# faithokamoto/panman

Measured on AMD Instinct MI355X. Metric: Fitch-Sankoff site*node updates/sec (fitch mode), higher is better.
Workload: dtype u32 bit-planes (16-bit one-hot state sets); 1 GPU; N* fitch: 1000000 leaves x 30000 sites random-join tree (one MI355X, north-star size); tree=random-join, leaves=1000000, nodes=1999999, sites=30000, sites_per_gpu=30000, parallelism=column shards x1, one all-gather of per-site score/root, gather=none (1 GPU), mutations_total=125584115, launch=hipGraph replay, per-level kernels

## Files before the change

### include/panman_gpu.h

```cpp
#ifndef PANMAN_GPU_H
#define PANMAN_GPU_H

#include <stdint.h>

#ifdef __cplusplus
extern "C" {
#endif

#define PM_OK 0
#define PM_ERR_ARG (-1)
#define PM_ERR_OOM (-2)
#define PM_ERR_HIP (-3)
#define PM_ERR_UNSUPPORTED (-4)
#define PM_ERR_STATE (-5)

#define PM_MODE_FITCH 0
#define PM_MODE_SANKOFF 1
#define PM_MODE_BLOCK_FITCH 2
#define PM_MODE_BLOCK_SANKOFF 3

#define PM_MUT_NS 0
#define PM_MUT_ND 1
#define PM_MUT_NI 2

typedef struct pm_ctx pm_ctx;

typedef struct pm_tree {
    int32_t num_nodes;
    int32_t root;
    const int32_t* child_offsets;
    const int32_t* child_index;
} pm_tree;

typedef struct pm_mut {
    uint32_t node;
    uint32_t site_info;
} pm_mut;

int pm_create(int device, pm_ctx** out);
void pm_destroy(pm_ctx* ctx);
int pm_warmup(int device);
const char* pm_last_error(const pm_ctx* ctx);
int pm_set_stream(pm_ctx* ctx, void* hip_stream);
#define PM_OPT_VIRTUAL 2
#define PM_OPT_GRAPH 3
#define PM_OPT_SUBTREE 6
#define PM_OPT_NARROW 7
#define PM_OPT_GROUP_WAVES 8
#define PM_OPT_GROUP_LEVELS 9
#define PM_OPT_UP_GROUP 10
#define PM_OPT_RECORD_CAP 12
#define PM_OPT_SUB_DOWN 13
#define PM_OPT_PLAIN_UP 14
#define PM_OPT_NT_LOADS 16
#define PM_OPT_CLUSTER 17
int pm_set_option(pm_ctx* ctx, int option, int64_t value);
int pm_set_profiling(pm_ctx* ctx, int enable);

int pm_tree_upload(pm_ctx* ctx, const pm_tree* tree);

int pm_leaves_upload(pm_ctx* ctx, int64_t num_sites, const uint8_t* codes4, int64_t row_stride,
                     const int32_t* node_row, const uint8_t* present, int64_t present_stride);

int pm_sites_upload(pm_ctx* ctx, const uint8_t* consensus4, const uint8_t* forced4);

int pm_run(pm_ctx* ctx, int mode);

int pm_mutation_count(pm_ctx* ctx, int64_t* count);
int pm_mutations_fetch(pm_ctx* ctx, pm_mut* out, int64_t cap, int64_t* count);
int pm_site_results(pm_ctx* ctx, int32_t* score, uint8_t* root_code);
int pm_site_results_device(pm_ctx* ctx, void* score_device, void* root_code_device);
int pm_kernel_times(pm_ctx* ctx, double* ms, int64_t* launches, int classes);

#define PM_COMM_ID_BYTES 128
int pm_comm_unique_id(uint8_t* id, int64_t len);
int pm_comm_init_rank(pm_ctx* ctx, const uint8_t* id, int nranks, int rank);
int pm_comm_init_all(pm_ctx* const* ctxs, int n);
int pm_run_gather(pm_ctx* ctx, int mode, int64_t total_sites, int64_t site_begin, void* score_device,
                  void* root_device);
int pm_multi_run(pm_ctx* const* ctxs, int n, int mode, const int64_t* site_begin, int64_t total_sites,
                 int32_t* score, uint8_t* root_code);
int pm_shard_range(int rank, int ranks, int64_t total_sites, int64_t* begin, int64_t* end);
int pm_pack_site_results(pm_ctx* ctx, int64_t site_begin, int64_t per, void* chunk_device);
int pm_unpack_site_results(pm_ctx* ctx, const void* all_device, int64_t per, int ranks, int64_t total_sites,
                           void* score_device, void* root_device);
int pm_chunk_entries(int64_t total_sites, int ranks, int64_t* per);
int pm_chunk_pack(int64_t site_begin, int64_t count, const int32_t* score, const uint8_t* root, int64_t per,
                  uint64_t* chunk);
int pm_chunk_unpack(const uint64_t* all, int64_t per, int ranks, int64_t total_sites, int32_t* score,
                    uint8_t* root);

int pm_design_bytes(pm_ctx* ctx, double* out, int n);
int pm_gather_probe(int device, int64_t lanes, int stride_bytes, int reps, double* ms_per_launch);
int pm_memory_footprint(pm_ctx* ctx, int64_t* out, int n);
const char* pm_build_id(void);
int pm_stream_copy_rate(int device, int64_t bytes, int reps, double* gbs);
int pm_stream_write_rate(int device, int64_t bytes, int reps, double* gbs);

void pm_phase_reset(void);
int64_t pm_phase_report(char* buf, int64_t len);

char* pm_msa_build(const char* newick, const char* msa_text, const char* reference, int mode, int device);
void pm_free(void* p);
int pm_msa_to_panman(const char* newick, const char* msa_text, const char* reference, int mode, int device,
                     const char* out_path, char* err, int64_t err_len);
int pm_msa_to_panman_multi(const char* newick, const char* msa_text, const char* reference, int mode,
                           const int* devices, int num_devices, const char* out_path, char* err, int64_t err_len);

// ... 82 lines not shown
```

### panman_amd/csrc/pm_fitch.hip

```cpp
#include "pm_kernels.h"

#if PM_NT_LOADS
#define launch_fitch launch_fitch_nt
#define warm_fitch warm_fitch_nt
#endif

namespace pm {
namespace {

#ifndef PM_LEAFY_WAVES
#define PM_LEAFY_WAVES 6
#endif
#ifndef PM_SUB_LEAFY_WAVES
#define PM_SUB_LEAFY_WAVES 4
#endif
#ifndef PM_SUB_UP_WAVES
#define PM_SUB_UP_WAVES 4
#endif
#ifndef PM_GROUP_UP_WAVES
#define PM_GROUP_UP_WAVES 4
#endif
template <bool AP, bool LEAFY, bool SUB = false, bool GROUP = false, bool PLAIN = false>
__device__ __forceinline__ void fitch_up_node(const UpArgs& a, const NodeDesc& d, int32_t gi, int tile, int lane) {
    constexpr bool SS = SUB && !PLAIN;
// ... 793 lines not shown
                else if (ap && c->group_waves > 0) hipLaunchKernelGGL((k_down_band<Mode::kFitch, true, false, true>), dim3(tiles), dim3(kBandBlock), 0, c->stream, dn, tab, base, d, d1);
                else if (ap) hipLaunchKernelGGL((k_down_band<Mode::kFitch, true>), dim3(tiles), dim3(kBandBlock), 0, c->stream, dn, tab, base, d, d1);
                else if (c->group_waves > 0) hipLaunchKernelGGL((k_down_band<Mode::kFitch, false, false, true>), dim3(tiles), dim3(kBandBlock), 0, c->stream, dn, tab, base, d, d1);
                else hipLaunchKernelGGL((k_down_band<Mode::kFitch, false>), dim3(tiles), dim3(kBandBlock), 0, c->stream, dn, tab, base, d, d1);
                timer_end(c, 1);
                d = d1 - 1;
                continue;
            }
        }
        dn.desc = down_desc + down_off[d];
        dn.count = down_off[d + 1] - down_off[d];
        if (dn.count == 0) continue;
        const bool dense = sub ? ht.down_dense_k : virt && ht.down_dense_v;
        dn.dense_base = !dense ? -1 : sub ? ht.down_dense_base_k[d] : down_off[d];
        auto narrow_down = [&](int l) { return c->narrow_max > 0 && down_off[l + 1] - down_off[l] <= c->narrow_max; };
        auto band_at = [&](int l) { return narrow_down(l) && l + 1 < D && narrow_down(l + 1); };
        int g = 1;
        int64_t items = dn.count;
        while (!block && c->group_waves > 0 && g < std::min(c->group_levels, kGroupLevels) && d + g < D) {
            const int32_t ng = down_off[d + g + 1] - down_off[d + g];
            if (ng == 0 || (items + ng) * tiles > c->group_waves || band_at(d + g)) break;
            items += ng;
            ++g;
        }
        if (g > 1) {
            for (int k = 0; k < 4; ++k) {
                const int l = std::min(d + k, d + g - 1);
                if (k > 0) dn.split[k - 1] = k < g ? down_off[d + k] - down_off[d] : (int32_t)items;
                dn.dense_g[k] = !dense ? -1 : sub ? ht.down_dense_base_k[l] : down_off[l];
            }
            dn.count = (int32_t)items;
            const dim3 grid = wave_grid(dn.count, tiles);
            timer_begin(c, 1);
            if (sub_down && dense) hipLaunchKernelGGL((k_down<Mode::kFitch, true, true, true, true>), grid, dim3(kBlock), 0, c->stream, dn);
            else if (sub_down) hipLaunchKernelGGL((k_down<Mode::kFitch, true, false, true, true>), grid, dim3(kBlock), 0, c->stream, dn);
            else if (ap && dense) hipLaunchKernelGGL((k_down<Mode::kFitch, true, true, false, true>), grid, dim3(kBlock), 0, c->stream, dn);
            else if (ap) hipLaunchKernelGGL((k_down<Mode::kFitch, true, false, false, true>), grid, dim3(kBlock), 0, c->stream, dn);
            else hipLaunchKernelGGL((k_down<Mode::kFitch, false, false, false, true>), grid, dim3(kBlock), 0, c->stream, dn);
            timer_end(c, 1);
            d += g - 1;
            continue;
        }
        const dim3 grid = wave_grid(dn.count, tiles);
        timer_begin(c, 1);
        if (block && ap) hipLaunchKernelGGL((k_down<Mode::kBlockFitch, true, false>), grid, dim3(kBlock), 0, c->stream, dn);
        else if (block) hipLaunchKernelGGL((k_down<Mode::kBlockFitch, false, false>), grid, dim3(kBlock), 0, c->stream, dn);
        else if (sub_down && dense) hipLaunchKernelGGL((k_down<Mode::kFitch, true, true, true>), grid, dim3(kBlock), 0, c->stream, dn);
        else if (sub_down) hipLaunchKernelGGL((k_down<Mode::kFitch, true, false, true>), grid, dim3(kBlock), 0, c->stream, dn);
        else if (ap && dense) hipLaunchKernelGGL((k_down<Mode::kFitch, true, true>), grid, dim3(kBlock), 0, c->stream, dn);
        else if (ap) hipLaunchKernelGGL((k_down<Mode::kFitch, true, false>), grid, dim3(kBlock), 0, c->stream, dn);
        else hipLaunchKernelGGL((k_down<Mode::kFitch, false, false>), grid, dim3(kBlock), 0, c->stream, dn);
        timer_end(c, 1);
    }
    const int32_t tail_skip = sub_down ? ht.num_tail_s : 0;
    const int32_t tail_total = (sub ? ht.num_tail_k : virt ? ht.num_tail_v : ht.num_tail) - tail_skip;
    if (tail_total > 0) {
        DownArgs t = dn;
        t.tail = (sub ? dt.tail_desc_k : virt ? dt.tail_desc_v : dt.tail_desc) + tail_skip;
        t.count = tail_total;
        t.num_s = sub && !sub_down ? ht.num_tail_s : 0;
        t.sbase = ht.sbase;
        t.sub_planes = c->sub_planes;
        const dim3 grid = wave_grid(t.count, tiles);
        timer_begin(c, 5);
        if (sub) hipLaunchKernelGGL((k_tail<Mode::kFitch, true, true>), grid, dim3(kBlock), 0, c->stream, t);
        else if (block && ap) hipLaunchKernelGGL((k_tail<Mode::kBlockFitch, true>), grid, dim3(kBlock), 0, c->stream, t);
        else if (block) hipLaunchKernelGGL((k_tail<Mode::kBlockFitch, false>), grid, dim3(kBlock), 0, c->stream, t);
        else if (ap) hipLaunchKernelGGL((k_tail<Mode::kFitch, true>), grid, dim3(kBlock), 0, c->stream, t);
        else hipLaunchKernelGGL((k_tail<Mode::kFitch, false>), grid, dim3(kBlock), 0, c->stream, t);
        timer_end(c, 5);
    }
    return hipGetLastError();
}

#if !PM_NT_LOADS
hipError_t launch_score(pm_ctx* c) {
    hipError_t e = hipMemsetAsync(c->score, 0, sizeof(int32_t) * c->num_sites, c->stream);
    if (e != hipSuccess) return e;
    const bool use_lds = c->num_sites * 4 <= 150 * 1024;
    const int spb = kShards >= 1024 ? kShards / 256 : 4;
    const int blocks = (kShards + spb - 1) / spb;
    const size_t lds = use_lds ? (size_t)c->num_sites * 4 : 0;
    timer_begin(c, 2);
    hipLaunchKernelGGL(k_site_score, dim3(blocks), dim3(kScoreBlock), lds, c->stream, c->recs, c->shard_cnt,
                       c->shard_cap, (uint32_t)c->ht.root, c->score, c->num_sites, spb, use_lds);
    timer_end(c, 2);
    return hipGetLastError();
}

#endif

hipError_t warm_fitch() {
    hipFuncAttributes at;
    return hipFuncGetAttributes(&at, reinterpret_cast<const void*>(&k_fitch_up_wide<true>));
}

}
```

### panman_amd/csrc/pm_host.cpp

```cpp
#include <algorithm>
#include <chrono>
#include <cstdio>
#include <cstdlib>
#include <random>
#include <cstring>
#include <numeric>
#include <string>
#include <vector>

#include "pm_internal.h"

namespace pm {

int fail(pm_ctx* c, int code, const std::string& msg) {
    if (c) c->err = msg;
    return code;
}

int hip_fail(pm_ctx* c, hipError_t e, const char* what) {
    return fail(c, PM_ERR_HIP, std::string(what) + ": " + hipGetErrorString(e));
}

namespace {

// ... 152 lines not shown
            if ((e = malloc_or_release(c, reinterpret_cast<void**>(&c->upm), need)) != hipSuccess)
                return fail(c, PM_ERR_OOM, std::string("up slots: ") + hipGetErrorString(e));
            c->upm_bytes = need;
        }
    }
    if (!fitch) {
        const size_t parts = (size_t)std::max(c->ht.part_off.empty() ? 0 : c->ht.part_off.back(),
                                              std::max(c->ht.part_off_v.empty() ? 0 : c->ht.part_off_v.back(),
                                                       std::max(c->ht.part_off_k.empty() ? 0 : c->ht.part_off_k.back(),
                                                                c->ht.part_off_gs.empty() ? 0 : c->ht.part_off_gs.back())));
        const size_t need = parts * kPartPlanes * wpad * sizeof(uint32_t);
        if (need > c->sk_parts_bytes) {
            dev_free(c->sk_parts);
            if ((e = malloc_or_release(c, reinterpret_cast<void**>(&c->sk_parts), need)) != hipSuccess)
                return fail(c, PM_ERR_OOM, std::string("Sankoff part counters: ") + hipGetErrorString(e));
            c->sk_parts_bytes = need;
        }
    }
    if (!c->shard_cnt && (e = dev_alloc(&c->shard_cnt, kShards)) != hipSuccess)
        return fail(c, PM_ERR_OOM, "shard counters");
    if (c->shard_cap == 0) {
        const double nodes = (double)c->dt.num_internal + c->dt.num_leaves;
        const double guess = std::max(65536.0, 0.01 * nodes * (double)c->num_sites);
        const int64_t cap = c->record_cap > 0 ? c->record_cap : (int64_t)(guess * 1.5 / kShards) + 256;
        if ((e = malloc_or_release(c, reinterpret_cast<void**>(&c->recs), sizeof(pm_mut) * (size_t)cap * kShards)) != hipSuccess)
            return fail(c, PM_ERR_OOM, std::string("mutation records: ") + hipGetErrorString(e));
        c->shard_cap = cap;
    }
    return PM_OK;
}

bool nt_policy(const pm_ctx* c) {
    if (c->nt_loads >= 0) return c->nt_loads != 0;
    const std::vector<int32_t>& off = c->ht.down_level_off;
    int64_t widest = 0;
    for (size_t l = 0; l + 1 < off.size(); ++l) widest = std::max<int64_t>(widest, off[l + 1] - off[l]);
    return widest * (wpad_of(c) / kWave) >= 65536;
}

hipError_t launch_all(pm_ctx* c, int mode) {
    const bool sankoff = mode == PM_MODE_SANKOFF || mode == PM_MODE_BLOCK_SANKOFF;
    const bool block = mode == PM_MODE_BLOCK_FITCH || mode == PM_MODE_BLOCK_SANKOFF;
    const bool nt = nt_policy(c);
    phase_add("run.nt_loads", nt ? 1.0 : 0.0);
    hipError_t e = sankoff ? (nt ? launch_sankoff_nt(c, block) : launch_sankoff(c, block))
                           : (nt ? launch_fitch_nt(c, block) : launch_fitch(c, block));
    if (e == hipSuccess) e = launch_score(c);
    return e;
}

uint64_t graph_key_of(const pm_ctx* c, int mode) {
    const uint64_t parts[] = {(uint64_t)mode, (uint64_t)c->virtual_leaf_parents, (uint64_t)c->subtree_form,
                              (uint64_t)c->narrow_max, (uint64_t)c->group_waves, (uint64_t)c->group_levels, (uint64_t)c->up_group,
                              (uint64_t)c->sub_down, (uint64_t)c->plain_up, (uint64_t)c->plain_min_waves, (uint64_t)c->cluster,
                              (uint64_t)(uintptr_t)c->upm,
                              (uint64_t)(uintptr_t)c->sk_parts,
                              (uint64_t)c->leaves_all_present, (uint64_t)c->has_forced, (uint64_t)c->num_sites,
                              (uint64_t)c->shard_cap, (uint64_t)(uintptr_t)c->recs, (uint64_t)(uintptr_t)c->sets,
                              (uint64_t)(uintptr_t)c->cmask, (uint64_t)(uintptr_t)c->root_final,
                              (uint64_t)(uintptr_t)c->leaf_planes, (uint64_t)(uintptr_t)c->leaf_present,
                              (uint64_t)(uintptr_t)c->leaf_flag, (uint64_t)(uintptr_t)c->cons,
                              (uint64_t)(uintptr_t)c->forced, (uint64_t)(uintptr_t)c->score,
                              (uint64_t)(uintptr_t)c->root_code, (uint64_t)(uintptr_t)c->shard_cnt,
                              (uint64_t)(uintptr_t)c->sub_planes, (uint64_t)nt_policy(c),
                              (uint64_t)(uintptr_t)c->dt.child_off, (uint64_t)(uintptr_t)c->stream};
    uint64_t h = 1469598103934665603ull;
    for (uint64_t v : parts) h = (h ^ v) * 1099511628211ull;
    return h | 1;
}

int run_once(pm_ctx* c, int mode) {
    hipError_t e;
    if (!c->use_graph) {
        e = launch_all(c, mode);
        if (e != hipSuccess) return hip_fail(c, e, "parsimony launch");
    } else {
        const uint64_t key = graph_key_of(c, mode);
        if (key != c->graph_key) {
            drop_graph(c);
            const bool prof = c->profiling;
            c->profiling = false;
            hipGraph_t g = nullptr;
            e = hipStreamBeginCapture(c->stream, hipStreamCaptureModeThreadLocal);
            if (e == hipSuccess) {
                const hipError_t le = launch_all(c, mode);
                e = hipStreamEndCapture(c->stream, &g);
                if (e == hipSuccess) e = le;
            }
            c->profiling = prof;
            if (e == hipSuccess) e = hipGraphInstantiate(&c->graph_exec, g, nullptr, nullptr, 0);
            if (g) (void)hipGraphDestroy(g);
            if (e != hipSuccess) {
                drop_graph(c);
                return hip_fail(c, e, "graph capture");
            }
            c->graph_key = key;
        }
        timer_begin(c, 4);
        e = hipGraphLaunch(c->graph_exec, c->stream);
        timer_end(c, 4);
        if (e != hipSuccess) return hip_fail(c, e, "graph launch");
    }
    c->ran = true;
    c->last_mode = mode;
    return PM_OK;
}

// ... 164 lines not shown
    free_columns(c);
    free_tree(c->dt);
    free_replay(c);
    comm_release(c);
    free_hostio(c);
    for (auto& v : c->timers)
        for (auto& t : v) {
            (void)hipEventDestroy(t.a);
            (void)hipEventDestroy(t.b);
        }
    if (c->side) (void)hipStreamSynchronize(c->side);
    if (c->ev_fork) (void)hipEventDestroy(c->ev_fork);
    if (c->ev_join) (void)hipEventDestroy(c->ev_join);
    if (c->side) (void)hipStreamDestroy(c->side);
    if (c->own_stream) (void)hipStreamDestroy(c->own_stream);
    delete c;
}

const char* pm_last_error(const pm_ctx* c) { return c ? c->err.c_str() : "null context"; }

int pm_set_stream(pm_ctx* c, void* s) {
    if (!c) return PM_ERR_ARG;
    c->stream = s ? reinterpret_cast<hipStream_t>(s) : c->own_stream;
    return PM_OK;
}

int pm_set_option(pm_ctx* c, int option, int64_t value) {
    if (!c) return PM_ERR_ARG;
    if (option == PM_OPT_SUBTREE) {
        c->subtree_form = value != 0;
        return PM_OK;
    }
    if (option == PM_OPT_VIRTUAL) {
        c->virtual_leaf_parents = value != 0;
        return PM_OK;
    }
    if (option == PM_OPT_NARROW) {
        if (value < 0 || value > 1024) return fail(c, PM_ERR_ARG, "PM_OPT_NARROW: 0..1024 items per level");
        c->narrow_max = (int32_t)value;
        return PM_OK;
    }
    if (option == PM_OPT_UP_GROUP) {
        c->up_group = value != 0;
        return PM_OK;
    }
    if (option == PM_OPT_PLAIN_UP) {
        if (value < 0) return fail(c, PM_ERR_ARG, "PM_OPT_PLAIN_UP: 0, 1 or a wave threshold >= 2");
        c->plain_up = value != 0;
        c->plain_min_waves = value >= 2 ? value : 0;
        return PM_OK;
    }
    if (option == PM_OPT_SUB_DOWN) {
        c->sub_down = value != 0;
        return PM_OK;
    }
    if (option == PM_OPT_GROUP_WAVES) {
        if (value < 0) return fail(c, PM_ERR_ARG, "PM_OPT_GROUP_WAVES: >= 0 waves");
        c->group_waves = value;
        return PM_OK;
    }
    if (option == PM_OPT_GROUP_LEVELS) {
        if (value < 2 || value > 4) return fail(c, PM_ERR_ARG, "PM_OPT_GROUP_LEVELS: 2 to 4");
        c->group_levels = (int32_t)value;
        return PM_OK;
    }
    if (option == PM_OPT_RECORD_CAP) {
        if (value < 1 || value > ((int64_t)1 << 31)) return fail(c, PM_ERR_ARG, "PM_OPT_RECORD_CAP: 1 .. 2^31 records per shard");
        if (c->stream) (void)hipStreamSynchronize(c->stream);
        drop_graph(c);
        dev_free(c->recs);
        c->shard_cap = 0;
        c->record_cap = value;
        c->ran = false;
        return PM_OK;
    }
    if (option == PM_OPT_NT_LOADS) {
        if (value < -1 || value > 1) return fail(c, PM_ERR_ARG, "PM_OPT_NT_LOADS: -1 (by level size), 0 or 1");
        c->nt_loads = (int32_t)value;
        return PM_OK;
    }
    if (option == PM_OPT_CLUSTER) {
        if (value < 0 || value > ((int64_t)1 << 30)) return fail(c, PM_ERR_ARG, "PM_OPT_CLUSTER: 0, 1 or a level size >= 2");
        c->cluster = value != 0;
        c->cluster_max_level = value == 0 ? 0 : value == 1 ? kClMaxLevel : (int32_t)value;
        c->cluster_chain = value == 1;
        return PM_OK;
    }
    if (option == PM_OPT_GRAPH) {
        c->use_graph = value != 0;
        if (!c->use_graph) drop_graph(c);
        return PM_OK;
    }
    return fail(c, PM_ERR_ARG, "unknown option");
}

int pm_set_profiling(pm_ctx* c, int enable) {
    if (!c) return PM_ERR_ARG;
    c->profiling = enable != 0;
    for (auto& u : c->timers_used) u = 0;
    return PM_OK;
}

int pm_tree_upload(pm_ctx* c, const pm_tree* t) {
    const bool timing = std::getenv("PM_UPLOAD_TIMING") != nullptr;
    auto t_last = std::chrono::steady_clock::now();
    auto upload_phase = [&](const char* what) {
// ... 979 lines not shown
```

### panman_amd/csrc/pm_internal.h

```cpp
#pragma once

#include <hip/hip_runtime.h>

#include <chrono>
#include <cstdint>
#include <functional>
#include <string>
#include <vector>

#include "../../include/panman_gpu.h"

namespace pm {

constexpr int kWave = 64;
constexpr int kWavesPerBlock = 4;
constexpr int kBlock = kWave * kWavesPerBlock;
#ifndef PM_SHARDS
#define PM_SHARDS 1024
#endif
constexpr int kShards = PM_SHARDS;
constexpr int kClasses = 6;
constexpr int kDegreeClasses = 4;
#ifndef PM_CX_COMPACT
#define PM_CX_COMPACT 0
// ... 156 lines not shown
    std::vector<int32_t> up_degree[4];
    std::vector<int32_t> up_level_off_k, up_class_off_k, down_level_off_k, down_dense_base_k;
    std::vector<uint8_t> up_leafy_k;
    std::vector<int32_t> up_level_off_g, up_class_off_g;
    std::vector<uint8_t> up_leafy_g, up_recomp_g;
    std::vector<int32_t> up_plain_g, up_plain_gs;
    std::vector<int32_t> up_level_off_gs, up_class_off_gs;
    std::vector<uint8_t> up_leafy_gs, up_recomp_gs;
    bool down_dense_k = false;
    int32_t up_items_k = 0, up_items_g = 0, up_items_gs = 0;
    int64_t num_sshape = 0;
    std::vector<uint8_t> sshape;
    int32_t num_tail_k = 0;
    int32_t num_tail_s = 0;
    int32_t sbase = -1;
    int64_t lvl_up[5] = {0, 0, 0, 0, 0}, lvl_down[3] = {0, 0, 0}, lvl_base_k = 0;
    ClusterPlan cl;
};

int plan_clusters(const HostTree& ht, const std::vector<int32_t>& up_order_k, const std::vector<int32_t>& child_enc_k,
                  const std::vector<int32_t>& parent_dense, const std::vector<int32_t>& vleaf, int32_t max_level,
                  bool chain_check, ClusterPlan& out);
bool plan_cluster_down(const HostTree& ht, const std::vector<int32_t>& down_order_k, const std::vector<NodeDesc>& down_desc_k,
                       const std::vector<int32_t>& child_enc_k, ClusterPlan& cl);

struct Timer {
    hipEvent_t a = nullptr, b = nullptr;
};

}

namespace pm { struct ReplayState; }

struct pm_ctx {
    int device = 0;
    hipStream_t stream = nullptr;
    hipStream_t own_stream = nullptr;
    hipStream_t side = nullptr;
    hipEvent_t ev_fork = nullptr, ev_join = nullptr;
    std::string err;

    pm::HostTree ht;
    pm::DevTree dt;
    size_t tree_bytes = 0;
    bool has_tree = false;
    int32_t max_degree = 0;
    bool virtual_leaf_parents = true;
    bool subtree_form = true;
    int32_t narrow_max = 16;
    int64_t group_waves = 32768;
    int32_t group_levels = 4;
    bool up_group = true;
    bool sub_down = false;
    bool plain_up = true;
    int64_t plain_min_waves = 0;
    bool cluster = true;
    int32_t cluster_max_level = pm::kClMaxLevel;
    bool cluster_chain = true;

    int64_t num_sites = 0;
    int32_t words = 0;
    uint4* leaf_planes = nullptr;
    uint32_t* leaf_present = nullptr;
    uint8_t* leaf_flag = nullptr;
    uint4* cons = nullptr;
    uint4* forced = nullptr;
    bool has_forced = false;
    bool has_leaves = false;
    bool leaves_all_present = false;
    bool has_sites = false;

    uint32_t* sets = nullptr;
    size_t sets_bytes = 0;
    uint64_t* cmask = nullptr;
    size_t cmask_bytes = 0;
    uint64_t* upm = nullptr;
    size_t upm_bytes = 0;
    uint4* finals = nullptr;
    size_t finals_bytes = 0;
    uint32_t* sk_parts = nullptr;
    size_t sk_parts_bytes = 0;
    uint4* root_final = nullptr;
    pm_mut* recs = nullptr;
    int64_t shard_cap = 0;
    int64_t record_cap = 0;
    uint32_t* shard_cnt = nullptr;
    uint4* sub_planes = nullptr;
    size_t sub_planes_bytes = 0;
    bool sub_planes_ok = false;
    int32_t* score = nullptr;
    uint8_t* root_code = nullptr;
    bool ran = false;
    int last_mode = -1;

    bool profiling = false;
    std::vector<pm::Timer> timers[pm::kClasses];
    size_t timers_used[pm::kClasses] = {0, 0, 0, 0, 0, 0};

    bool use_graph = false;
    int32_t nt_loads = -1;
    hipGraphExec_t graph_exec = nullptr;
    uint64_t graph_key = 0;

    pm::ReplayState* replay = nullptr;

    void* comm = nullptr;
// ... 149 lines not shown
```

### panman_amd/csrc/pm_kernels.h

```cpp
#pragma once

#include "pm_bits.h"
#include "pm_internal.h"

#ifndef PM_NT_LOADS
#define PM_NT_LOADS 0
#endif
#if PM_NT_LOADS
#define PM_KNS kern_nt
#else
#define PM_KNS kern
#endif

namespace pm {
inline namespace PM_KNS {

enum class Mode { kFitch, kSankoff, kBlockFitch };

#ifndef PM_TILE_FAST
#define PM_TILE_FAST 1
#endif
__device__ __forceinline__ void wave_item(int wave, int32_t tiles, int32_t& item, int& tile) {
#if PM_TILE_FAST
    const int32_t g = (int32_t)blockIdx.x * kWavesPerBlock + wave;
// ... 1113 lines not shown
        r.H = r.F;
    } else {
        const uint4 D = k.L3;
        const uint32_t ia = ~code_ne(A, Cc) | ~code_ne(A, D), ib = ~code_ne(B, Cc) | ~code_ne(B, D), nz = ia | ib;
        const uint32_t hit = (nz & ((ePa & ia) | (ePb & ib))) | (~nz & (ePa | ePb | ePc | ~code_ne(P, D)));
        const uint4 mcd = min4(Cc, D);
        r.F = sel4(hit, P, sel4(nz, sel4(ia & ib, mab, sel4(ia, A, B)), min4(mab, mcd)));
        r.H = sel4(~code_ne(r.F, Cc) | ~code_ne(r.F, D), r.F, mcd);
    }
    r.G = sel4(~code_ne(r.F, A) | ~code_ne(r.F, B), r.F, mab);
    return r;
}

__device__ __forceinline__ uint4 cherry_final_sankoff(const uint4& A, const uint4& B, const uint4& F) {
    const uint4 mab = min4(A, B);
    const uint4 open = sel4(~code_ne(F, A) | ~code_ne(F, B), F, min4(mab, F));
    return sel4(~code_ne(A, B), A, open);
}

__device__ __forceinline__ SubFinals subtree_finals_sankoff(const Kid& k, int sh, const uint4& P) {
    const uint4 A = k.L0, B = k.L1, Cc = k.L2;
    const uint4 mab = min4(A, B);
    const uint32_t pX = ~code_ne(P, A) | ~code_ne(P, B);
    SubFinals r;
    if (sh == 1) {
        const uint32_t inx = ~code_ne(Cc, A) | ~code_ne(Cc, B);
        const uint4 f_in = sel4(pX & code_less(&P.x, &Cc.x), P, Cc);
        const uint4 f_out = sel4(pX | ~code_ne(P, Cc), P, min4(min4(mab, Cc), P));
        r.F = sel4(inx, f_in, f_out);
        r.H = r.F;
    } else {
        const uint4 D = k.L3;
        const uint4 mcd = min4(Cc, D);
        const uint32_t ia = ~code_ne(A, Cc) | ~code_ne(A, D), ib = ~code_ne(B, Cc) | ~code_ne(B, D), nz = ia | ib;
        const uint32_t pY = ~code_ne(P, Cc) | ~code_ne(P, D);
        const uint32_t p_z0 = (~code_ne(P, A) & ia) | (~code_ne(P, B) & ib);
        const uint4 low = sel4(ia & ib, mab, sel4(ia, A, B));
        const uint4 f_nz = sel4(p_z0 | ((pX ^ pY) & code_less(&P.x, &low.x)), P, low);
        const uint4 f_z = sel4(pX | pY, P, min4(min4(mab, mcd), P));
        r.F = sel4(nz, f_nz, f_z);
        r.H = cherry_final_sankoff(Cc, D, r.F);
    }
    r.G = cherry_final_sankoff(A, B, r.F);
    return r;
}

template <class Args>
__device__ __forceinline__ void emit_code(const Args& a, Emit& em, int lane, uint32_t node, uint32_t D, uint32_t site0,
                                          const uint4& c, const uint4& pc) {
    const uint32_t p4[4] = {pc.x, pc.y, pc.z, pc.w};
    emit_stream(a, em, lane, node, D, site0, c.x, c.y, c.z, c.w, p4);
}

template <Mode M, class Args>
__device__ __forceinline__ void subtree_emit(const Args& a, Emit& em, int lane, const int32_t* id, int32_t ix, int32_t iy,
                                             const Kid& k, int sh, uint32_t valid, const uint32_t* Fn, uint32_t site0) {
    const uint4 P = make_uint4(Fn[0], Fn[1], Fn[2], Fn[3]);
    const SubFinals f = M == Mode::kSankoff ? subtree_finals_sankoff(k, sh, P) : subtree_finals(k, sh, P);
    const uint32_t msk = valid & k.m0;
    emit_code(a, em, lane, (uint32_t)id[0], msk & code_ne(f.F, P), site0, f.F, P);
    emit_code(a, em, lane, (uint32_t)ix, msk & code_ne(f.G, f.F), site0, f.G, f.F);
    emit_code(a, em, lane, (uint32_t)id[1], msk & code_ne(k.L0, f.G), site0, k.L0, f.G);
    emit_code(a, em, lane, (uint32_t)id[2], msk & code_ne(k.L1, f.G), site0, k.L1, f.G);
    const uint4 pc = sh == 1 ? f.F : f.H;
    emit_code(a, em, lane, (uint32_t)id[3], msk & code_ne(k.L2, pc), site0, k.L2, pc);
    if (sh == 2) {
        emit_code(a, em, lane, (uint32_t)iy, msk & code_ne(f.H, f.F), site0, f.H, f.F);
        emit_code(a, em, lane, (uint32_t)id[4], msk & code_ne(k.L3, f.H), site0, k.L3, f.H);
    }
}

template <Mode M, class Args>
__device__ __forceinline__ void kid_emit(const Args& a, Emit& em, int lane, const Kid& k, uint32_t id0, uint32_t id1,
                                         uint32_t id2, uint32_t valid, const uint32_t* Fn, uint32_t site0) {
    if (k.enc < 0) {
        emit_stream(a, em, lane, id0, valid & k.m0 & diff4(k.L0, Fn), site0, k.L0.x, k.L0.y, k.L0.z, k.L0.w, Fn);
        return;
    }
    if (M == Mode::kBlockFitch || !(k.enc & kVirtualBit)) return;
    uint32_t low[4] = {0, 0, 0, 0}, have = 0, hit = 0;
    virt_fold(k.L0, k.m0, Fn, low, have, hit);
    virt_fold(k.L1, k.m1, Fn, low, have, hit);
    if (M == Mode::kSankoff) {
        const uint32_t z1_has_fn =
            (k.m0 ^ k.m1) |
            (k.m0 & k.m1 & ((k.L0.x ^ k.L1.x) | (k.L0.y ^ k.L1.y) | (k.L0.z ^ k.L1.z) | (k.L0.w ^ k.L1.w)));
        const uint32_t take = z1_has_fn & code_less(Fn, low);
#pragma unroll
        for (int j = 0; j < 4; ++j) low[j] = bsel(take, Fn[j], low[j]);
    }
    uint32_t F[4];
#pragma unroll
    for (int j = 0; j < 4; ++j) F[j] = bsel(hit, Fn[j], low[j]);
    const uint32_t self = have & valid & ((F[0] ^ Fn[0]) | (F[1] ^ Fn[1]) | (F[2] ^ Fn[2]) | (F[3] ^ Fn[3]));
    emit_stream(a, em, lane, id0, self, site0, F[0], F[1], F[2], F[3], Fn);
    emit_stream(a, em, lane, id1, valid & k.m0 & diff4(k.L0, F), site0, k.L0.x, k.L0.y, k.L0.z, k.L0.w, F);
    if (k.vl.y >= 0)
        emit_stream(a, em, lane, id2, valid & k.m1 & diff4(k.L1, F), site0, k.L1.x, k.L1.y, k.L1.z, k.L1.w, F);
}

__device__ __forceinline__ uint32_t final_slot(const RecMask& m) {
    return (uint32_t)__builtin_popcountll(m.s) + lanes_below(m.x);
}

__device__ __forceinline__ uint4 rec_final(const uint4* p, const RecMask& m, int lane, const uint4* cons, int64_t word) {
    const uint4* src = ((m.x >> lane) & 1ull) ? p + final_slot(m)
                                              : ((m.s >> lane) & 1ull) ? p + lanes_below(m.s) : cons + word;
    return *src;
}

template <int REC>
__device__ __forceinline__ uint4 parent_final(const DownArgs& a, int32_t parent, const RecMask& m, int tile, int lane,
                                              int64_t word) {
    if (parent == a.root_dense) return a.root_final[word];
    const RecMask pm{m.px, m.ps, 0, 0, 0};
    return rec_final(a.sets + ((size_t)parent * a.tiles + tile) * REC, pm, lane, a.cons, word);
}

template <int REC>
__device__ __forceinline__ uint4 node_final(const DownArgs& a, int32_t node, int tile, int lane, int64_t word) {
    if (node == a.root_dense) return a.root_final[word];
// ... 151 lines not shown
        kid_emit<M>(a, em, lane, kids[1], kids[1].id0, kids[1].id1, kids[1].id2, valid, F, site0);
    }
    emit_flush<M != Mode::kSankoff>(a, em, lane);
}

template <Mode M, bool AP, bool DENSE, bool SUB = false, bool GROUP = false>
#ifndef PM_SK_GROUP_WAVES
#define PM_SK_GROUP_WAVES 7
#endif
#ifndef PM_DOWN_WAVES
#define PM_DOWN_WAVES 8
#endif
#ifndef PM_SK_DOWN_WAVES
#define PM_SK_DOWN_WAVES 6
#endif
__global__ __launch_bounds__(kBlock, GROUP ? (M == Mode::kSankoff ? PM_SK_GROUP_WAVES : SUB ? PM_SUB_DOWN_WAVES : 8) : SUB ? PM_SUB_DOWN_WAVES : (M == Mode::kFitch && AP) ? PM_DOWN_WAVES : (M == Mode::kSankoff && AP) ? PM_SK_DOWN_WAVES : 1) void k_down(DownArgs a) {
    __shared__ uint4 stage[kWavesPerBlock][kEntryQuads];
    const int wave = __builtin_amdgcn_readfirstlane(threadIdx.x >> 6), lane = threadIdx.x & 63;
    int32_t item;
    int tile;
    wave_item(wave, a.tiles, item, tile);
    if (item >= a.count) return;
    const NodeDesc& d = a.desc[item];
    const int gen = !GROUP ? 0 : (item >= a.split[0]) + (item >= a.split[1]) + (item >= a.split[2]);
    const int32_t first = gen == 0 ? 0 : a.split[gen > 0 ? gen - 1 : 0];
    const int32_t n = !DENSE ? d.node : (GROUP ? a.dense_g[gen] : a.dense_base) + (item - first);
    down_node<M, AP, SUB, GROUP>(a, d, n, (uint32_t)item, tile, lane, stage[wave], gen);
}

template <Mode M, bool AP, bool SUB = false, bool GROUP = false>
__global__ __launch_bounds__(kBandBlock) void k_down_band(DownArgs a, const int32_t* level_off, const int32_t* dense_base,
                                                          int32_t d0, int32_t d1) {
    __shared__ uint4 stage[kBandWaves][kEntryQuads];
    const int wave = __builtin_amdgcn_readfirstlane(threadIdx.x >> 6), lane = threadIdx.x & 63;
    const int tile = blockIdx.x;
    constexpr int G = GROUP ? kGroupLevels : 1;
    for (int32_t l0 = d0; l0 < d1; l0 += G) {
        const int32_t l1 = min(l0 + G, d1);
        for (int32_t i = level_off[l0] + wave; i < level_off[l1]; i += kBandWaves) {
            int32_t l = l0;
            while (l + 1 < l1 && i >= level_off[l + 1]) ++l;
            const NodeDesc& d = a.desc[i];
            const int32_t base = dense_base ? dense_base[l] : -1;
            down_node<M, AP, SUB, GROUP>(a, d, base >= 0 ? base + (i - level_off[l]) : d.node, (uint32_t)i, tile, lane,
                                         stage[wave], l - l0);
        }
        __syncthreads();
    }
}

#ifndef PM_TAIL_WAVES
#define PM_TAIL_WAVES 6
#endif
template <Mode M, bool AP, bool SUB = false>
__global__ __launch_bounds__(kBlock, SUB ? PM_TAIL_WAVES : 1) void k_tail(DownArgs a) {
    __shared__ uint4 stage[kWavesPerBlock][kEntryQuads];
    const int wave = __builtin_amdgcn_readfirstlane(threadIdx.x >> 6), lane = threadIdx.x & 63;
    int32_t item;
    int tile;
    wave_item(wave, a.tiles, item, tile);
    if (item >= a.count) return;
    const TailDesc& t = a.tail[item];
    const int64_t word = (int64_t)tile * kWave + lane;
    const uint32_t valid = valid_mask(a, word);
    constexpr int REC = M == Mode::kSankoff ? kSankoffRec : kFitchRec;
    RecMask pm;
    bool proot;
    if (SUB && item < a.num_s) {
        const uint64_t* q = a.cmask + kMaskWords * ((size_t)(a.sbase + item) * a.tiles + tile);
        pm = RecMask{q[3], q[4], q[5], 0, 0};
        if (pm.d == 0) return;
        proot = t.parent == a.root_dense;
    } else {
        proot = t.parent == a.root_dense;
        pm = rec_mask(a.cmask, (size_t)t.parent * a.tiles + tile);
        if (leaf_rule<M, AP>(t.enc)) pm.d = pm.x;
        if (!proot && pm.d == 0) return;
    }
    const size_t prec = (size_t)t.parent * a.tiles + tile;
    const bool dirty = proot || ((pm.d >> lane) & 1ull);
    Kid k;
    if (SUB && item < a.num_s) {
        k.enc = t.enc;
        k.L0 = k.L1 = k.L2 = k.L3 = make_uint4(0, 0, 0, 0);
        k.m0 = k.m1 = 0;
        const uint4* q = sub_word(a.sub_planes, item, a.wpad, word);
        if (dirty) {
            k.L0 = q[0];
            k.L1 = q[1];
            k.L2 = q[2];
            k.m0 = k.m1 = ~0u;
        }
        if (dirty && kid_shape(t.enc) == 2) k.L3 = q[3];
    } else {
        kid_fetch<M, AP, SUB, false>(a, t.enc, make_int4(t.vl[0], t.vl[1], t.vl[2], t.vl[3]), word, dirty, k);
    }
    const uint4* fsrc = proot ? a.root_final + word
                              : ((pm.x >> lane) & 1ull) ? a.sets + prec * REC + final_slot(pm)
                              : ((pm.s >> lane) & 1ull) ? a.sets + prec * REC + lanes_below(pm.s) : a.cons + word;
    uint4 q = make_uint4(0, 0, 0, 0);
    if (dirty) q = *fsrc;
    const uint32_t F[4] = {q.x, q.y, q.z, q.w};
    Emit em{stage[wave], shard_of((uint32_t)item, tile), 0u, 0u};
    const uint32_t site0 = (uint32_t)(word * 32);
    if (SUB && kid_shape(t.enc)) subtree_emit<M>(a, em, lane, t.id, t.ix, t.iy, k, kid_shape(t.enc), valid, F, site0);
    else kid_emit<M>(a, em, lane, k, (uint32_t)t.id[0], (uint32_t)t.id[1], (uint32_t)t.id[2], valid, F, site0);
    emit_flush<M != Mode::kSankoff>(a, em, lane);
}

struct ClArgs {
    const NodeDesc* items;
    const int32_t* wg_off;
    const int32_t* slot_of;
    const int32_t* pslot;
// ... 241 lines not shown
```

### panman_amd/engine.py

```python
from __future__ import annotations

import ctypes as C

import numpy as np

from ._lib import MODE_BLOCK_FITCH, MODE_BLOCK_SANKOFF, MODE_FITCH, MODE_SANKOFF, Mut, PanmanError, Summary, Tree, load

CLUSTER_DEFAULT = 1

__all__ = ["Engine", "msa_build", "random_join_tree", "pack_codes", "MODE_FITCH", "MODE_SANKOFF"]


def pack_codes(codes: np.ndarray) -> np.ndarray:
    codes = np.ascontiguousarray(codes, dtype=np.uint8)
    if codes.ndim == 1:
        return pack_codes(codes[None, :])[0]
    rows, s = codes.shape
    if s % 2:
        codes = np.concatenate([codes, np.zeros((rows, 1), np.uint8)], axis=1)
    return np.ascontiguousarray(codes[:, 0::2] | (codes[:, 1::2] << 4))


def random_join_tree(leaves: int, seed: int = 1):
    lib = load()
# ... 162 lines not shown
    dv = (C.c_int * len(devices))(*devices)
    n = C.c_int64(0)
    err = C.create_string_buffer(512)
    rc = lib.pm_fasta_multi_fd(C.byref(st), int(aligned), dv, len(devices), int(fd), C.byref(n), err, len(err))
    del keep
    if rc != 0:
        raise PanmanError(f"pm_fasta_multi_fd failed ({rc}): {err.value.decode(errors='replace')}")
    return n.value


class Engine:
    def __init__(self, device: int = 0):
        self.lib = load()
        self.ctx = C.c_void_p()
        rc = self.lib.pm_create(device, C.byref(self.ctx))
        if rc != 0:
            raise PanmanError(f"pm_create({device}) failed ({rc}): no usable HIP device")
        self.num_sites = 0

    def close(self):
        if self.ctx:
            self.lib.pm_destroy(self.ctx)
            self.ctx = C.c_void_p()

    def __del__(self):
        try:
            self.close()
        except Exception:
            pass

    def _check(self, rc: int, what: str):
        if rc != 0:
            msg = self.lib.pm_last_error(self.ctx)
            raise PanmanError(f"{what}: rc={rc}: {msg.decode() if msg else ''}")

    def set_stream(self, stream_handle: int):
        self._check(self.lib.pm_set_stream(self.ctx, C.c_void_p(stream_handle)), "pm_set_stream")

    def set_virtual(self, on: bool):
        self._check(self.lib.pm_set_option(self.ctx, 2, int(on)), "pm_set_option")

    def set_subtree(self, on: bool):
        self._check(self.lib.pm_set_option(self.ctx, 6, int(on)), "pm_set_option")

    def set_narrow(self, max_items: int):
        self._check(self.lib.pm_set_option(self.ctx, 7, int(max_items)), "pm_set_option")

    def set_group(self, max_waves: int, levels: int = 4):
        self._check(self.lib.pm_set_option(self.ctx, 8, int(max_waves)), "pm_set_option")
        self._check(self.lib.pm_set_option(self.ctx, 9, int(levels)), "pm_set_option")

    def set_sub_down(self, on: bool):
        self._check(self.lib.pm_set_option(self.ctx, 13, int(on)), "pm_set_option")

    def set_plain_up(self, on: bool, min_waves: int = 0):
        value = (int(min_waves) if min_waves >= 2 else 1) if on else 0
        self._check(self.lib.pm_set_option(self.ctx, 14, value), "pm_set_option")

    def set_up_group(self, on: bool):
        self._check(self.lib.pm_set_option(self.ctx, 10, int(on)), "pm_set_option")

    def set_record_cap(self, records_per_shard: int):
        self._check(self.lib.pm_set_option(self.ctx, 12, int(records_per_shard)), "pm_set_option")

    def set_nt_loads(self, value: int):
        self._check(self.lib.pm_set_option(self.ctx, 16, int(value)), "pm_set_option")

    def set_cluster(self, value: int):
        self._check(self.lib.pm_set_option(self.ctx, 17, int(value)), "pm_set_option")

    def set_graph(self, on: bool):
        self._check(self.lib.pm_set_option(self.ctx, 3, int(on)), "pm_set_option")

    def set_profiling(self, on: bool):
        self._check(self.lib.pm_set_profiling(self.ctx, int(on)), "pm_set_profiling")

    def tree_upload(self, child_offsets, child_index, root: int):
        self._off = np.ascontiguousarray(child_offsets, dtype=np.int32)
        self._idx = np.ascontiguousarray(child_index, dtype=np.int32)
        t = Tree(self._off.shape[0] - 1, int(root), self._off.ctypes.data, self._idx.ctypes.data)
        self._check(self.lib.pm_tree_upload(self.ctx, C.byref(t)), "pm_tree_upload")

    def leaves_upload(self, codes: np.ndarray, node_row, present: np.ndarray | None = None):
        codes = np.ascontiguousarray(codes, dtype=np.uint8)
        s = codes.shape[1]
        packed = pack_codes(codes)
        node_row = np.ascontiguousarray(node_row, dtype=np.int32)
        pp, pstride = None, 0
        if present is not None:
            bits = np.packbits(np.ascontiguousarray(present, dtype=bool), axis=1, bitorder="little")
            bits = np.ascontiguousarray(bits)
            pp, pstride = bits.ctypes.data, bits.shape[1]
            self._keep_present = bits
        self._check(self.lib.pm_leaves_upload(self.ctx, s, packed.ctypes.data, packed.shape[1],
                                              node_row.ctypes.data, pp, pstride), "pm_leaves_upload")
        self.num_sites = s

    def sites_upload(self, consensus: np.ndarray, forced: np.ndarray | None = None):
        c4 = pack_codes(np.asarray(consensus, dtype=np.uint8))
        f4 = pack_codes(np.asarray(forced, dtype=np.uint8)) if forced is not None else None
        self._check(self.lib.pm_sites_upload(self.ctx, c4.ctypes.data,
                                             f4.ctypes.data if f4 is not None else None),
                    "pm_sites_upload")

    def synth_columns(self, site_begin: int, num_sites: int, seed: int = 2):
        self._check(self.lib.pm_synth_columns(self.ctx, site_begin, num_sites, seed), "pm_synth_columns")
# ... 171 lines not shown
```

Before: 4273 billion site*node updates/s.

## Pack sparse subtree tail items into compacted waves via per-wave lane scan

```diff
diff --git a/include/panman_gpu.h b/include/panman_gpu.h
--- a/include/panman_gpu.h
+++ b/include/panman_gpu.h
@@ -54,6 +54,7 @@
 #define PM_OPT_PLAIN_UP 14
 #define PM_OPT_NT_LOADS 16
 #define PM_OPT_CLUSTER 17
+#define PM_OPT_TAIL_PACK 18
 int pm_set_option(pm_ctx* ctx, int option, int64_t value);
 int pm_set_profiling(pm_ctx* ctx, int enable);
 
diff --git a/panman_amd/csrc/pm_fitch.hip b/panman_amd/csrc/pm_fitch.hip
--- a/panman_amd/csrc/pm_fitch.hip
+++ b/panman_amd/csrc/pm_fitch.hip
@@ -869,13 +869,30 @@
         else hipLaunchKernelGGL((k_down<Mode::kFitch, false, false>), grid, dim3(kBlock), 0, c->stream, dn);
         timer_end(c, 1);
     }
-    const int32_t tail_skip = sub_down ? ht.num_tail_s : 0;
+    const int64_t pack_min = c->tail_pack_min_waves != 0 ? c->tail_pack_min_waves : kTailPackMinWaves;
+    const bool pack = sub && !sub_down && c->tail_pack && ht.num_tail_s > 0 && (int64_t)ht.num_tail_s * tiles >= pack_min;
+    constexpr int G = kTailPack;
+    phase_add("run.tail_pack", pack ? (double)G : 0.0);
+    phase_add("run.tail_s_waves", sub ? (double)ht.num_tail_s * tiles : 0.0);
+    if (pack) {
+        DownArgs t = dn;
+        t.tail = dt.tail_desc_k;
+        t.num_s = ht.num_tail_s;
+        t.count = (ht.num_tail_s + G - 1) / G;
+        t.sbase = ht.sbase;
+        t.sub_planes = c->sub_planes;
+        const dim3 grid = wave_grid(t.count, tiles);
+        timer_begin(c, 5);
+        hipLaunchKernelGGL((k_tail<Mode::kFitch, true, true, G>), grid, dim3(kBlock), 0, c->stream, t);
+        timer_end(c, 5);
+    }
+    const int32_t tail_skip = sub_down || pack ? ht.num_tail_s : 0;
     const int32_t tail_total = (sub ? ht.num_tail_k : virt ? ht.num_tail_v : ht.num_tail) - tail_skip;
     if (tail_total > 0) {
         DownArgs t = dn;
         t.tail = (sub ? dt.tail_desc_k : virt ? dt.tail_desc_v : dt.tail_desc) + tail_skip;
         t.count = tail_total;
-        t.num_s = sub && !sub_down ? ht.num_tail_s : 0;
+        t.num_s = sub && !sub_down && !pack ? ht.num_tail_s : 0;
         t.sbase = ht.sbase;
         t.sub_planes = c->sub_planes;
         const dim3 grid = wave_grid(t.count, tiles);
diff --git a/panman_amd/csrc/pm_host.cpp b/panman_amd/csrc/pm_host.cpp
--- a/panman_amd/csrc/pm_host.cpp
+++ b/panman_amd/csrc/pm_host.cpp
@@ -228,7 +228,7 @@
 uint64_t graph_key_of(const pm_ctx* c, int mode) {
     const uint64_t parts[] = {(uint64_t)mode, (uint64_t)c->virtual_leaf_parents, (uint64_t)c->subtree_form,
                               (uint64_t)c->narrow_max, (uint64_t)c->group_waves, (uint64_t)c->group_levels, (uint64_t)c->up_group,
-                              (uint64_t)c->sub_down, (uint64_t)c->plain_up, (uint64_t)c->plain_min_waves, (uint64_t)c->cluster,
+                              (uint64_t)c->sub_down, (uint64_t)c->tail_pack, (uint64_t)c->tail_pack_min_waves, (uint64_t)c->plain_up, (uint64_t)c->plain_min_waves, (uint64_t)c->cluster,
                               (uint64_t)(uintptr_t)c->upm,
                               (uint64_t)(uintptr_t)c->sk_parts,
                               (uint64_t)c->leaves_all_present, (uint64_t)c->has_forced, (uint64_t)c->num_sites,
@@ -499,6 +499,12 @@
     }
     if (option == PM_OPT_SUB_DOWN) {
         c->sub_down = value != 0;
+        return PM_OK;
+    }
+    if (option == PM_OPT_TAIL_PACK) {
+        if (value < -1) return fail(c, PM_ERR_ARG, "PM_OPT_TAIL_PACK: -1, 0, 1 or a wave threshold >= 2");
+        c->tail_pack = value != 0;
+        c->tail_pack_min_waves = value >= 2 ? value : value < 0 ? -1 : 0;
         return PM_OK;
     }
     if (option == PM_OPT_GROUP_WAVES) {
diff --git a/panman_amd/csrc/pm_internal.h b/panman_amd/csrc/pm_internal.h
--- a/panman_amd/csrc/pm_internal.h
+++ b/panman_amd/csrc/pm_internal.h
@@ -232,6 +232,8 @@
     int32_t group_levels = 4;
     bool up_group = true;
     bool sub_down = false;
+    bool tail_pack = true;
+    int64_t tail_pack_min_waves = 0;
     bool plain_up = true;
     int64_t plain_min_waves = 0;
     bool cluster = true;
diff --git a/panman_amd/csrc/pm_kernels.h b/panman_amd/csrc/pm_kernels.h
--- a/panman_amd/csrc/pm_kernels.h
+++ b/panman_amd/csrc/pm_kernels.h
@@ -1189,7 +1189,7 @@
     emit_stream(a, em, lane, node, D, site0, c.x, c.y, c.z, c.w, p4);
 }
 
-template <Mode M, class Args>
+template <Mode M, bool LANES = false, class Args>
 __device__ __forceinline__ void subtree_emit(const Args& a, Emit& em, int lane, const int32_t* id, int32_t ix, int32_t iy,
                                              const Kid& k, int sh, uint32_t valid, const uint32_t* Fn, uint32_t site0) {
     const uint4 P = make_uint4(Fn[0], Fn[1], Fn[2], Fn[3]);
@@ -1201,9 +1201,10 @@
     emit_code(a, em, lane, (uint32_t)id[2], msk & code_ne(k.L1, f.G), site0, k.L1, f.G);
     const uint4 pc = sh == 1 ? f.F : f.H;
     emit_code(a, em, lane, (uint32_t)id[3], msk & code_ne(k.L2, pc), site0, k.L2, pc);
-    if (sh == 2) {
-        emit_code(a, em, lane, (uint32_t)iy, msk & code_ne(f.H, f.F), site0, f.H, f.F);
-        emit_code(a, em, lane, (uint32_t)id[4], msk & code_ne(k.L3, f.H), site0, k.L3, f.H);
+    if (LANES || sh == 2) {
+        const uint32_t m3 = sh == 2 ? msk : 0u;
+        emit_code(a, em, lane, (uint32_t)iy, m3 & code_ne(f.H, f.F), site0, f.H, f.F);
+        emit_code(a, em, lane, (uint32_t)id[4], m3 & code_ne(k.L3, f.H), site0, k.L3, f.H);
     }
 }
 
@@ -1461,14 +1462,116 @@
 #ifndef PM_TAIL_WAVES
 #define PM_TAIL_WAVES 6
 #endif
-template <Mode M, bool AP, bool SUB = false>
-__global__ __launch_bounds__(kBlock, SUB ? PM_TAIL_WAVES : 1) void k_tail(DownArgs a) {
+#ifndef PM_TAIL_PACK
+#define PM_TAIL_PACK 8
+#endif
+#ifndef PM_TAIL_PACK_WAVES
+#define PM_TAIL_PACK_WAVES 6
+#endif
+constexpr int kTailPack = PM_TAIL_PACK;
+#ifndef PM_TAIL_PACK_MIN_WAVES
+#define PM_TAIL_PACK_MIN_WAVES 65536
+#endif
+constexpr int64_t kTailPackMinWaves = PM_TAIL_PACK_MIN_WAVES;
+constexpr int kPackInfoQuads = 4;
+
+__device__ __forceinline__ uint32_t bits_below(uint64_t m, uint32_t l) {
+    return (uint32_t)__builtin_popcountll(m & ((1ull << l) - 1ull));
+}
+
+template <Mode M, int G>
+__device__ __forceinline__ void tail_packed(const DownArgs& a, int32_t group, int tile, int lane, uint4* stage, uint4* info,
+                                            uint16_t* slots) {
+    constexpr int REC = M == Mode::kSankoff ? kSankoffRec : kFitchRec;
+    const int32_t item0 = group * G;
+    const int32_t mine = item0 + lane;
+    const bool own = lane < G && mine < a.num_s;
+    uint64_t px = 0, ps = 0, md = 0;
+    uint4 d0 = make_uint4(0, 0, 0, 0), d2 = make_uint4(0, 0, 0, 0);
+    uint32_t id4 = 0;
+    if (own) {
+        const uint64_t* q = a.cmask + kMaskWords * ((size_t)(a.sbase + mine) * a.tiles + tile);
+        px = q[3];
+        ps = q[4];
+        md = q[5];
+        const uint4* tp = reinterpret_cast<const uint4*>(a.tail + mine);
+        d0 = tp[0];
+        d2 = tp[2];
+        id4 = (uint32_t)a.tail[mine].id[4];
+    }
+    if (own && (int32_t)d0.x == a.root_dense) md = ~0ull;
+    uint32_t T;
+    const uint32_t pre = wave_exclusive_scan((uint32_t)__builtin_popcountll(md), T);
+    if (T == 0) return;
+    if (lane < G) {
+        uint4* w = info + lane * kPackInfoQuads;
+        w[0] = d0;
+        w[1] = d2;
+        w[2] = make_uint4(id4, 0u, 0u, 0u);
+        w[3] = make_uint4((uint32_t)px, (uint32_t)(px >> 32), (uint32_t)ps, (uint32_t)(ps >> 32));
+    }
+#pragma unroll
+    for (int g = 0; g < G; ++g) {
+        const uint32_t lo = __builtin_amdgcn_readlane((uint32_t)md, g), hi = __builtin_amdgcn_readlane((uint32_t)(md >> 32), g);
+        const uint64_t m = (uint64_t)lo | ((uint64_t)hi << 32);
+        const uint32_t p = __builtin_amdgcn_readlane(pre, g);
+        if ((m >> lane) & 1ull) slots[p + lanes_below(m)] = (uint16_t)(g * kWave + lane);
+    }
+    __builtin_amdgcn_wave_barrier();
+    Emit em{stage, shard_of((uint32_t)group, tile), 0u, 0u};
+    for (uint32_t r0 = 0; r0 < T; r0 += kWave) {
+        const uint32_t j = r0 + (uint32_t)lane;
+        const bool act = j < T;
+        const uint32_t slot = slots[act ? j : r0];
+        const uint32_t g = slot >> 6, l = slot & 63u;
+        const uint4* w = info + g * kPackInfoQuads;
+        const uint4 i0 = w[0], i1 = w[1], i2 = w[2], i3 = w[3];
+        const int32_t parent = (int32_t)i0.x, enc = (int32_t)i0.y;
+        const int sh = kid_shape(enc);
+        const int64_t word = (int64_t)tile * kWave + l;
+        const uint32_t valid = act ? valid_mask(a, word) : 0u;
+        Kid k;
+        k.enc = enc;
+        k.L0 = k.L1 = k.L2 = k.L3 = make_uint4(0, 0, 0, 0);
+        k.m0 = k.m1 = 0;
+        const uint4* q = sub_word(a.sub_planes, item0 + (int32_t)g, a.wpad, word);
+        if (act) {
+            k.L0 = q[0];
+            k.L1 = q[1];
+            k.L2 = q[2];
+            k.m0 = k.m1 = ~0u;
+        }
+        if (act && sh == 2) k.L3 = q[3];
+        const uint64_t mx = (uint64_t)i3.x | ((uint64_t)i3.y << 32), ms = (uint64_t)i3.z | ((uint64_t)i3.w << 32);
+        const uint4* pb = a.sets + ((size_t)parent * a.tiles + tile) * REC;
+        const uint4* fsrc = parent == a.root_dense ? a.root_final + word
+                            : ((mx >> l) & 1ull)   ? pb + (uint32_t)__builtin_popcountll(ms) + bits_below(mx, l)
+                            : ((ms >> l) & 1ull)   ? pb + bits_below(ms, l)
+                                                   : a.cons + word;
+        uint4 pf = make_uint4(0, 0, 0, 0);
+        if (act) pf = *fsrc;
+        const uint32_t F[4] = {pf.x, pf.y, pf.z, pf.w};
+        const int32_t id[5] = {(int32_t)i1.x, (int32_t)i1.y, (int32_t)i1.z, (int32_t)i1.w, (int32_t)i2.x};
+        subtree_emit<M, true>(a, em, lane, id, (int32_t)i0.z, (int32_t)i0.w, k, sh, valid, F, (uint32_t)(word * 32));
+    }
+    emit_flush<M != Mode::kSankoff>(a, em, lane);
+}
+
+template <Mode M, bool AP, bool SUB = false, int G = 0>
+__global__ __launch_bounds__(kBlock, G > 0 ? PM_TAIL_PACK_WAVES : SUB ? PM_TAIL_WAVES : 1) void k_tail(DownArgs a) {
     __shared__ uint4 stage[kWavesPerBlock][kEntryQuads];
     const int wave = __builtin_amdgcn_readfirstlane(threadIdx.x >> 6), lane = threadIdx.x & 63;
     int32_t item;
     int tile;
     wave_item(wave, a.tiles, item, tile);
     if (item >= a.count) return;
+    if constexpr (G > 0) {
+        static_assert(SUB && AP && G <= kWave && G * kWave <= 65536, "packed tail: S2 / S3 items, slot = g * 64 + lane in 16 bits");
+        __shared__ uint4 info[kWavesPerBlock][G * kPackInfoQuads];
+        __shared__ uint16_t slots[kWavesPerBlock][G * kWave];
+        tail_packed<M, G>(a, item, tile, lane, stage[wave], info[wave], slots[wave]);
+        return;
+    }
     const TailDesc& t = a.tail[item];
     const int64_t word = (int64_t)tile * kWave + lane;
     const uint32_t valid = valid_mask(a, word);
diff --git a/panman_amd/engine.py b/panman_amd/engine.py
--- a/panman_amd/engine.py
+++ b/panman_amd/engine.py
@@ -238,6 +238,9 @@
 
     def set_sub_down(self, on: bool):
         self._check(self.lib.pm_set_option(self.ctx, 13, int(on)), "pm_set_option")
+
+    def set_tail_pack(self, value: int):
+        self._check(self.lib.pm_set_option(self.ctx, 18, int(value)), "pm_set_option")
 
     def set_plain_up(self, on: bool, min_waves: int = 0):
         value = (int(min_waves) if min_waves >= 2 else 1) if on else 0
```

New measurement: 4553 billion site*node updates/s (median of 6 runs). 6.5% higher.
